# maxdoblas/QuickEd

Hardware: AMD Instinct MI355X
Metric: alignments/sec + GCUPS, 10kb x 10kb 5%-error pairs (higher is better)
Workload: dtype u64; 1 GPU; banded_score, DEVICE-RESIDENT inputs: 100000 pairs/GPU x 10000 bp @ 0.05 error, bandwidth 15 %, seeded generator (SURVEY 8d), ASCII already in HBM when the clock starts, results left in HBM (end-to-end rates: e2e); pairs_per_gpu=100000, length=10000, bandwidth=15, parallelism=pairs sharded over 1 GPU(s), no data-path collective

## Files before the change

### quicked_amd/capi.py

```python
import ctypes as C
import os

import numpy as np

from . import build

QUICKED, WINDOWED, BANDED, HIRSCHBERG = 0, 1, 2, 3
QUICKED_OK, QUICKED_ERROR, QUICKED_FAIL_NON_CONVERGENCE = 0, -1, -2
QUICKED_UNKNOWN_ALGO, QUICKED_EMPTY_SEQUENCE, QUICKED_UNIMPLEMENTED, QUICKED_WIP = -3, -4, -10, 1


class ProfilerCounter(C.Structure):
    _fields_ = [("total", C.c_uint64), ("samples", C.c_uint64), ("min", C.c_uint64), ("max", C.c_uint64),
                ("m_oldM", C.c_double), ("m_newM", C.c_double), ("m_oldS", C.c_double), ("m_newS", C.c_double)]


class Timespec(C.Structure):
    _fields_ = [("tv_sec", C.c_long), ("tv_nsec", C.c_long)]


class ProfilerTimer(C.Structure):
    _fields_ = [("begin_timer", Timespec), ("time_ns", ProfilerCounter), ("accumulated", C.c_uint64)]


# ... 92 lines not shown
    L.quicked_batch_hits.restype = C.c_int
    L.quicked_batch_run_panel.argtypes = [C.c_void_p, C.c_int, C.c_int32, C.c_void_p, C.c_void_p, C.c_void_p, C.c_void_p, C.c_int32, C.c_int]
    L.quicked_batch_run_panel.restype = C.c_int
    L.quicked_batch_panel_results.argtypes = [C.c_void_p, C.c_void_p]
    L.quicked_batch_panel_results.restype = C.c_int
    L.quicked_batch_panel_matrix.argtypes = [C.c_void_p, C.c_void_p, C.c_void_p]
    L.quicked_batch_panel_matrix.restype = C.c_int
    L.quicked_batch_run_panel_all.argtypes = [C.c_void_p, C.c_int, C.c_int32, C.c_void_p, C.c_void_p, C.c_void_p, C.c_void_p, C.c_int32, C.c_int32, C.c_int]
    L.quicked_batch_run_panel_all.restype = C.c_int
    L.quicked_batch_panel_hit_counts.argtypes = [C.c_void_p, C.c_void_p, C.c_void_p]
    L.quicked_batch_panel_hit_counts.restype = C.c_int
    L.quicked_batch_panel_hit_total.argtypes = [C.c_void_p]
    L.quicked_batch_panel_hit_total.restype = C.c_int64
    L.quicked_batch_panel_hits.argtypes = [C.c_void_p, C.c_void_p, C.c_void_p]
    L.quicked_batch_panel_hits.restype = C.c_int
    L.quicked_batch_sync.argtypes = [C.c_void_p]
    L.quicked_batch_scores.argtypes = [C.c_void_p, C.c_void_p, C.c_void_p]
    L.quicked_batch_cigar_bytes.restype = C.c_int64
    L.quicked_batch_cigar_bytes.argtypes = [C.c_void_p]
    L.quicked_batch_cigars.argtypes = [C.c_void_p, C.c_void_p, C.c_void_p]
    L.quicked_batch_counters.argtypes = [C.c_void_p, C.c_void_p]
    L.quicked_batch_kernel_time.argtypes = [C.c_void_p, C.POINTER(C.c_double), C.POINTER(C.c_int64)]
    if hasattr(L, "quicked_batch_kernel_times"):
        L.quicked_batch_kernel_times.argtypes = [C.c_void_p, C.c_void_p, C.c_void_p]
    L.quicked_batch_configure.argtypes = [C.c_void_p, C.c_int, C.c_int]
    L.quicked_batch_check_results.argtypes = [C.c_void_p, C.c_void_p]
    L.quicked_batch_validate.argtypes = [C.c_void_p, C.c_char_p, C.c_int64, C.c_void_p, C.c_void_p]
    L.quicked_batch_configure_tags.argtypes = [C.c_void_p, C.c_int]
    L.quicked_batch_pair_stats.argtypes = [C.c_void_p, C.c_void_p]
    L.quicked_batch_md_bytes.restype = C.c_int64
    L.quicked_batch_md_bytes.argtypes = [C.c_void_p]
    L.quicked_batch_md.argtypes = [C.c_void_p, C.c_void_p, C.c_void_p]
    L.quicked_debug_tag_launches.argtypes = [C.c_void_p]
    L.quicked_wire_words.restype = C.c_int64
    L.quicked_wire_words.argtypes = [C.c_int32, C.c_int]
    L.quicked_wire_pack.argtypes = [C.c_char_p, C.c_int32, C.c_int, C.c_void_p]
    L.quicked_batch_create_packed.restype = C.c_void_p
    L.quicked_batch_create_packed.argtypes = [C.c_int64, C.c_int, C.c_void_p, C.c_void_p, C.c_void_p, C.c_void_p, C.c_void_p, C.c_void_p]
    L.quicked_batch_reload.argtypes = [C.c_void_p, C.c_int64, C.c_void_p, C.c_void_p, C.c_void_p, C.c_void_p, C.c_void_p, C.c_void_p]
    L.quicked_batch_reload_packed.argtypes = [C.c_void_p, C.c_int64, C.c_int, C.c_void_p, C.c_void_p, C.c_void_p, C.c_void_p, C.c_void_p, C.c_void_p]
    L.quicked_batch_fetch.argtypes = [C.c_void_p]
    L.quicked_pool_stats.argtypes = [C.c_void_p]
    if hasattr(L, "quicked_early_finish_stats"):
        L.quicked_early_finish_stats.argtypes = [C.c_void_p]
    L.quicked_batch_cigar_view.argtypes = [C.c_void_p, C.POINTER(C.c_void_p), C.POINTER(C.c_void_p)]
    L.quicked_batch_deferred_pairs.restype = C.c_int64
    L.quicked_batch_deferred_pairs.argtypes = [C.c_void_p]
    L.quicked_wire_pack_pool.argtypes = [C.c_int64, C.c_void_p, C.c_void_p, C.c_void_p, C.c_int, C.c_void_p, C.c_void_p, C.c_int,
                                         C.POINTER(C.c_int64)]
    L.quicked_wire_offsets.restype = C.c_int64
    L.quicked_wire_offsets.argtypes = [C.c_int64, C.c_void_p, C.c_int, C.c_void_p]
    L.quicked_wire_pack_isa.argtypes = [C.c_int]
    L.quicked_host_alloc.restype = C.c_void_p
    L.quicked_host_alloc.argtypes = [C.c_size_t]
    L.quicked_host_free.argtypes = [C.c_void_p]
    L.quicked_host_free.restype = None
    _LIB = L
    return L


def reload_env():
    if _LIB is not None and hasattr(_LIB, "quicked_debug_reload_env"):
        _LIB.quicked_debug_reload_env()


def tag_launches():
    v = np.zeros(2, dtype=np.int64)
    lib().quicked_debug_tag_launches(v.ctypes.data)
    return int(v[0]), int(v[1])


def pool_trim():
    return lib().quicked_pool_trim()


def pool_stats():
    v = np.zeros(8, dtype=np.int64)
    lib().quicked_pool_stats(v.ctypes.data)
    return dict(pool_bytes=int(v[0]), reclaim_events=int(v[1]), sets=int(v[2]), sub_batches=int(v[3]), pool_budget=int(v[4]),
                device_pool_bytes=int(v[5]), contexts=int(v[6]), contexts_leased=int(v[7]))


def early_finish_stats():
    v = np.zeros(4, dtype=np.int64)
    lib().quicked_early_finish_stats(v.ctypes.data)
    return dict(flows=int(v[0]), batches=int(v[1]), merged_flows=int(v[2]), merged_batches=int(v[3]))


def make_params(**kw):
    p = lib().quicked_default_params()
    for k, v in kw.items():
        if k in ("hew_threshold", "hew_percentage"):
            getattr(p, k)[0], getattr(p, k)[1] = v
        else:
            setattr(p, k, v)
    return p


class QuickedException(Exception):
    def __init__(self, status):
        self.status = status
        super().__init__(lib().quicked_status_msg(status).decode())


# ... 399 lines not shown
```

### quicked_amd/csrc/qe_batch.h

```cpp
#pragma once
#include <hip/hip_runtime.h>

#include <condition_variable>
#include <cstdint>
#include <cstring>
#include <memory>
#include <mutex>
#include <vector>

#include "quicked.h"
#include "quicked_batch.h"
#include "qe_types.h"
#include "qe_pool.h"

struct quicked_batch {
    int64_t n = 0;
    int device = 0;
    std::vector<int32_t> p_len, t_len;
    std::vector<int64_t> p_off, t_off;
    std::vector<int64_t> plp_off, plt_off;
    std::vector<int32_t> order;
    uint8_t* arena = nullptr;
    size_t arena_bytes = 0;
    uint8_t *d_asc_p = nullptr, *d_asc_t = nullptr;
// ... 117 lines not shown
    t->accumulated += ns;
    profiler_counter_t* c = &t->time_ns;
    const uint64_t amount = t->accumulated;
    c->total += amount;
    ++c->samples;
    if (c->samples == 1) { c->min = amount; c->max = amount; c->m_oldM = (double)amount; c->m_newM = (double)amount; c->m_oldS = 0.0; }
    else {
        c->min = std::min(c->min, amount); c->max = std::max(c->max, amount);
        c->m_newM = c->m_oldM + ((double)amount - c->m_oldM) / (double)c->samples;
        c->m_newS = c->m_oldS + ((double)amount - c->m_oldM) * ((double)amount - c->m_newM);
        c->m_oldM = c->m_newM; c->m_oldS = c->m_newS;
    }
    t->accumulated = 0;
}

inline double now_ms() { return mono_ms(); }
inline bool trace_on() { return sw_set(Sw::Trace); }
#define QE_TRACE_POINT(name) do { if (qe::trace_on()) { double t__ = qe::now_ms(); fprintf(stderr, "[qe t%03d @%.1f] %-22s +%.3f ms\n", (int)(syscall(SYS_gettid) % 1000), t__, name, t__ - tr_last); tr_last = t__; } } while (0)

struct BoundedRun { const int32_t* max_dist; int32_t max_dist_all; };
struct PanelRun { int32_t n_patterns; const char* pool; const int64_t* off; const int32_t* len; bool matrix; };
struct SearchRun { int mode; const int32_t* max_dist; int32_t max_dist_all; int32_t max_hits = 0; int eq = 0; const PanelRun* panel = nullptr; };
quicked_status_t run_batch(quicked_batch& B, const quicked_params_t& p, bool fetch, const BoundedRun* bd = nullptr, const SearchRun* sr = nullptr);
quicked_status_t fetch_results(quicked_batch& B);
void batch_load(quicked_batch* B, Context& C, int64_t n,
                const char* pattern_pool, const int64_t* pattern_off, const int32_t* pattern_len,
                const char* text_pool, const int64_t* text_off, const int32_t* text_len);
void batch_load_packed(quicked_batch* B, Context& C, int64_t n, int wire,
                       const uint64_t* pattern_words, const int64_t* pattern_word_off, const int32_t* pattern_len,
                       const uint64_t* text_words, const int64_t* text_word_off, const int32_t* text_len);
void batch_quiesce(quicked_batch* B);
void finisher_retire();
quicked_status_t batch_validate(quicked_batch* B, Context& C, const char* cigar_pool, int64_t pool_bytes, const int64_t* cigar_off, int32_t* ok_out);
void early_finish_stats(int64_t stats_out[4]);
int64_t tag_launches(int form);

}
```

### quicked_amd/csrc/qe_capi.cpp

```cpp
#include <hip/hip_runtime.h>

#include <algorithm>
#include <cstdio>
#include <cstdlib>
#include <cstring>
#include <functional>
#include <mutex>
#include <string>
#include <unordered_map>
#include <vector>

#include "qe_batch.h"
#include "qe_panel.h"

#define QE_API extern "C" __attribute__((visibility("default")))

using namespace qe;

QE_API void* quicked_host_alloc(size_t bytes) {
    void* p = nullptr;
    if (hipHostMalloc(&p, bytes, hipHostMallocDefault) != hipSuccess) return nullptr;
    return p;
}
QE_API void quicked_host_free(void* p) { if (p) (void)hipHostFree(p); }
// ... 463 lines not shown
    for (int q = 0; q < 8; ++q) stats_out[q] = 0;
    for (const auto& bk : g_book) stats_out[1] += bk.oom_events.load();
    Context* C = tl_ctx;
    const int dev = C ? C->device : tl_device;
    if (dev >= 0 && dev < QE_MAX_DEVICES) stats_out[5] = (int64_t)g_book[dev].held.load();
    { std::lock_guard<std::mutex> lk(g_ctx_mu); for (const Context* c : g_ctx_all) { ++stats_out[6]; if (c->leased.load()) ++stats_out[7]; } }
    if (!C) return QUICKED_OK;
    stats_out[0] = (int64_t)C->held.load();
    stats_out[2] = C->last_na; stats_out[3] = C->last_sub_batches; stats_out[4] = (int64_t)C->pool_budget;
    return QUICKED_OK;
}

QE_API quicked_status_t quicked_pool_trim(void) {
    finisher_retire();
    ApiScope scope;
    try {
        Context& C = ctx();
        (void)C.release_pools(nullptr, true);
        C.release_small_pinned();
        { std::lock_guard<std::mutex> lk(g_ctx_mu); C.planned = 0; C.wanted = 0; }
        (void)release_unleased(C.device);
        retire_idle_streams(C.device);
        return QUICKED_OK;
    } catch (const HipError& e) {
        fprintf(stderr, "[quicked_hip] HIP error %d (%s) at %s, qe_driver.hip:%d\n", (int)e.e, hipGetErrorString(e.e), e.what, e.line);
        return QUICKED_ERROR;
    }
}

QE_API quicked_status_t quicked_debug_tag_launches(int64_t out[2]) {
    if (!out) return QUICKED_ERROR;
    out[0] = qe::tag_launches(0); out[1] = qe::tag_launches(1);
    return QUICKED_OK;
}

QE_API quicked_status_t quicked_debug_reload_env(void) {
    qe::switches_reload();
    {
        std::lock_guard<std::mutex> lk(qe::g_ctx_mu);
        for (qe::Context* c : qe::g_ctx_all) {
            for (auto& v : c->narrow_off) v = 0;
            for (auto& ring : c->narrow_q) for (auto& v : ring) v = 0;
        }
    }
    return QUICKED_OK;
}

QE_API quicked_status_t quicked_early_finish_stats(int64_t stats_out[4]) {
    qe::early_finish_stats(stats_out);
    return QUICKED_OK;
}

QE_API int64_t quicked_batch_deferred_pairs(quicked_batch_t* batch) { return batch ? batch->res[batch->vis].deferred_pairs : -1; }

QE_API quicked_status_t quicked_batch_counters(quicked_batch_t* batch, int64_t counters_out[8]) {
    memcpy(counters_out, batch->res[batch->vis].counters, sizeof(batch->counters));
    return QUICKED_OK;
}

QE_API bool quicked_check_error(quicked_status_t status) { return status < 0; }

QE_API const char* quicked_status_msg(quicked_status_t status) {
    switch (status) {
        case QUICKED_ERROR: return "ERROR: QuickEd has finished with unspecific error\n";
        case QUICKED_FAIL_NON_CONVERGENCE: return "ERROR: Hirschberg algorithm can not find a middle point of subsequence division!\n";
        case QUICKED_UNIMPLEMENTED: return "ERROR: The algorithm or parameter combination selected is not implemented\n";
// ... 181 lines not shown
```

### quicked_amd/csrc/qe_driver.hip

```cpp
#include <hip/hip_runtime.h>

#include <algorithm>
#include <atomic>
#include <chrono>
#include <condition_variable>
#include <deque>
#include <cstdio>
#include <unistd.h>
#include <cstdlib>
#include <cstring>
#include <functional>
#include <memory>
#include <mutex>
#include <unordered_map>
#include <numeric>
#include <string>
#include <thread>
#include <vector>

#include "quicked.h"
#include "quicked_batch.h"
#include "qe_types.h"
#include "qe_pool.h"
#include "qe_batch.h"
// ... 1583 lines not shown
    }
    HIP_CHECK(hipStreamSynchronize(C.stream));
    QE_TRACE_POINT("load_packed: arrays");
    B->d_wire_p = d_pw; B->d_wire_t = d_tw; B->d_wire_p_off = d_pwo; B->d_wire_t_off = d_two;
    B->unpack_pending = n > 0; B->unpack_event_set = false;
    if (!B->ev_unpacked) HIP_CHECK(hipEventCreateWithFlags(&B->ev_unpacked, hipEventDisableTiming));
    HIP_CHECK(hipStreamSynchronize(C.stream));
}
}

namespace qe {
quicked_status_t fetch_results(quicked_batch& B) { return fetch_pending(B); }
void early_finish_stats(int64_t stats_out[4]) { for (int q = 0; q < 4; ++q) stats_out[q] = g_fin_stats[q].load(); }

quicked_status_t batch_validate(quicked_batch* B, Context& C, const char* cigar_pool, int64_t pool_bytes, const int64_t* cigar_off, int32_t* ok_out) {
    for (int64_t i = 0; i < B->n; ++i) if (cigar_off[i] >= pool_bytes) return QUICKED_ERROR;
    C.sync_all();
    C.phase_u();
    const DevicePool::Mark mk = C.pool_w.mark();
    char* d_pool = C.pool_w.take<char>((size_t)pool_bytes + 16);
    int64_t* d_off = C.pool_w.take<int64_t>((size_t)B->n + 1);
    int32_t* d_ok = C.pool_w.take<int32_t>((size_t)B->n + 1);
    if (pool_bytes > 0) HIP_CHECK(hipMemcpyAsync(d_pool, cigar_pool, (size_t)pool_bytes, hipMemcpyHostToDevice, C.stream));
    HIP_CHECK(hipMemsetAsync(d_pool + pool_bytes, 0, 16, C.stream));
    HIP_CHECK(hipMemcpyAsync(d_off, cigar_off, (size_t)B->n * sizeof(int64_t), hipMemcpyHostToDevice, C.stream));
    const int blocks = (int)((B->n + 63) / 64);
    hipLaunchKernelGGL(k_check_strings, dim3(blocks), dim3(64), 0, C.stream, pair_view(*B, false), (int)B->n,
                       (const char*)d_pool, (const int64_t*)d_off, d_ok);
    HIP_CHECK(hipMemcpyAsync(ok_out, d_ok, (size_t)B->n * sizeof(int32_t), hipMemcpyDeviceToHost, C.stream));
    HIP_CHECK(hipStreamSynchronize(C.stream));
    C.pool_w.release(mk);
    return QUICKED_OK;
}
}
```

### quicked_amd/csrc/qe_kernels.hip

```cpp
#include <type_traits>
#include <hip/hip_runtime.h>
#include "qe_types.h"
#include "qe_bounded.h"
#include "qe_search.h"
#include "qe_panel.h"
#include "qe_tags.h"
#include "qe_check.h"

namespace qe {

#define QE_ONES (~(u64)0)
#define QE_WAVE_IN_BLOCK() ((int)(threadIdx.x >> 6))
#define QE_GROUP_INDEX() ((int)(blockIdx.x * (blockDim.x >> 6) + (threadIdx.x >> 6)))
extern __shared__ uint4 qe_dyn_lds[];

__device__ __forceinline__ u32 lo32(u64 x) { return (u32)x; }
__device__ __forceinline__ u32 hi32(u64 x) { return (u32)(x >> 32); }
__device__ __forceinline__ u64 mk64(u32 lo, u32 hi) { return ((u64)hi << 32) | lo; }

__device__ __forceinline__ int64_t tile_elem(int col, int slot, int nslots) {
    return ((int64_t)(col >> 3) * nslots + slot) * 512 + (col & 7);
}

__device__ __forceinline__ int wave_min(int v) {
#pragma unroll
    for (int o = 32; o > 0; o >>= 1) v = min(v, __shfl_xor(v, o));
    return v;
}
__device__ __forceinline__ int wave_max(int v) {
#pragma unroll
    for (int o = 32; o > 0; o >>= 1) v = max(v, __shfl_xor(v, o));
    return v;
}

__device__ __forceinline__ void block_step(u64 Eq, u64& P, u64& M, u32 PHin, u32 MHin, u64& Ph_raw, u64& Mh_raw) {
    const u64 Xv = Eq | M;
    const u64 Eqc = Eq | (u64)MHin;
    const u64 Xh = (((Eqc & P) + P) ^ P) | Eqc;
// ... 581 lines not shown
            x[k] = (r0 >> sh) | (r1 << (64 - sh));
            y[k] = (r1 >> sh) | (r2 << (64 - sh));
        } else { x[k] = r0; y[k] = r1; }
    }
}

__device__ __forceinline__ void load_planes_ab(const u64* __restrict__ base, int bit, u64& a, u64& b) {
    const int w = bit >> 6, sh = bit & 63, o = sh ? 3 : 0;
    const u64* q = base + 3 * (int64_t)w;
    const u64 a0 = q[0], b0 = q[1], a1 = q[o], b1 = q[o + 1];
    a = (a0 >> sh) | ((a1 << 1) << (63 - sh));
    b = (b0 >> sh) | ((b1 << 1) << (63 - sh));
}

__device__ __forceinline__ void planes_ab_raw(const u64* __restrict__ base, int bit, u64 (&w)[4]) {
    const int o = (bit & 63) ? 3 : 0;
    const u64* q = base + 3 * (int64_t)(bit >> 6);
    w[0] = q[0]; w[1] = q[1]; w[2] = q[o]; w[3] = q[o + 1];
}
__device__ __forceinline__ void planes_ab_finish(const u64 (&w)[4], int bit, u64& a, u64& b) {
    const int sh = bit & 63;
    a = (w[0] >> sh) | ((w[2] << 1) << (63 - sh));
    b = (w[1] >> sh) | ((w[3] << 1) << (63 - sh));
}
struct TbsFetch { int q, Rb, cf_a, cf_b, cl_b; uint4 c0, w0; u64 t[4], p[4]; };

__device__ __forceinline__ int plane_code(const u64* __restrict__ base, int pos) {
    const u64* q = base + 3 * (int64_t)(pos >> 6);
    const int s = pos & 63;
    if ((q[2] >> s) & 1) return 4;
    return (int)(((q[0] >> s) & 1) | (((q[1] >> s) & 1) << 1));
}

__device__ __forceinline__ u32 gather_msb4(u32 x) {
    u32 t = (x << 7) | x;
    t = (x << 14) | t;
    return (x << 21) | t;
}

__global__ __launch_bounds__(256) void k_pack(PackArgs A) {
    const int lane = threadIdx.x & 63;
    const int seq = blockIdx.x * 4 + (threadIdx.x >> 6);
    if (seq >= A.nseq) return;
    const int len = A.len[seq];
    const uint8_t* __restrict__ src = A.asc + A.asc_off[seq];
    u64* __restrict__ dst = A.planes + A.pl_off[seq];
    const int nrows = ((len + 63) >> 6) + 2;
    const int nspan = (nrows + 15) >> 4;
    u32 fl = 0;
    constexpr int UNR = 4;
    constexpr u32 ALL_A = 0x41414141u;
    for (int s0 = 0; s0 < nspan; s0 += UNR) {
        uint4 raw[UNR];
#pragma unroll
        for (int u = 0; u < UNR; ++u) {
            const int pos = (s0 + u) * 1024 + 16 * lane;
            uint4 x = make_uint4(ALL_A, ALL_A, ALL_A, ALL_A);
            if (pos + 16 <= len) {
                if (A.reverse) {
                    uint4 y; __builtin_memcpy(&y, src + (len - 16 - pos), 16);
                    x = make_uint4(__builtin_bswap32(y.w), __builtin_bswap32(y.z), __builtin_bswap32(y.y), __builtin_bswap32(y.x));
                } else {
                    __builtin_memcpy(&x, src + pos, 16);
                }
            } else if (pos < len) {
                u32 wv[4] = {ALL_A, ALL_A, ALL_A, ALL_A};
                for (int i = 0; i < len - pos; ++i) {
                    const u32 c = A.reverse ? src[len - 1 - pos - i] : src[pos + i];
                    wv[i >> 2] = (wv[i >> 2] & ~(0xFFu << (8 * (i & 3)))) | (c << (8 * (i & 3)));
                }
                x = make_uint4(wv[0], wv[1], wv[2], wv[3]);
            }
            raw[u] = x;
        }
#pragma unroll
        for (int u = 0; u < UNR; ++u) {
            const int span = s0 + u;
            if (span >= nspan) break;
            const u32 wv[4] = {raw[u].x, raw[u].y, raw[u].z, raw[u].w};
            u32 accA = 0, accB = 0, accN = 0;
#pragma unroll
            for (int k = 0; k < 4; ++k) {
                const u32 w = wv[k];
                const u32 want = __builtin_amdgcn_perm(0u, 0x47544341u, (w >> 1) & 0x03030303u);
                const u32 y = want ^ (w & 0xDFDFDFDFu);
                const u32 z = ((y & 0x7F7F7F7Fu) + 0x7F7F7F7Fu) | y;
                const u32 ok = ~z & 0x80808080u, bad = z & 0x80808080u;
                accA = (accA >> 4) | (gather_msb4((w << 6) & ok) & 0xF0000000u);
                accB = (accB >> 4) | (gather_msb4((w << 5) & ok) & 0xF0000000u);
                accN = (accN >> 4) | (gather_msb4(bad) & 0xF0000000u);
                if ((w << 2) & ok) fl |= FLAG_NONCANON;
                if (bad) {
                    fl |= FLAG_HAS_N;
                    for (int i = 0; i < 4; ++i)
                        if (((bad >> (8 * i + 7)) & 1) && ((w >> (8 * i)) & 0xFF) != 'N') fl |= FLAG_NONCANON;
                }
            }
            const u32 ab = (accA >> 16) | (accB & 0xFFFF0000u), nn = accN >> 16;
            const u32 ab1 = __shfl_down(ab, 1), nn1 = __shfl_down(nn, 1);
            const u32 a32 = (ab & 0xFFFFu) | (ab1 << 16), b32 = (ab >> 16) | (ab1 & 0xFFFF0000u), n32 = nn | (nn1 << 16);
            const u32 a32h = __shfl_down(a32, 2), b32h = __shfl_down(b32, 2), n32h = __shfl_down(n32, 2);
            const int row = span * 16 + (lane >> 2);
            if ((lane & 3) == 0 && row < nrows) {
                u64* q = dst + 3 * (int64_t)row;
                q[0] = mk64(a32, a32h); q[1] = mk64(b32, b32h); q[2] = mk64(n32, n32h);
            }
        }
    }
    if (A.flags && __any(fl != 0)) {
        u32 f = fl;
#pragma unroll
        for (int o = 32; o > 0; o >>= 1) f |= __shfl_xor(f, o);
        if (lane == 0) atomicOr(&A.flags[seq], f);
    }
}

__device__ __forceinline__ u32 even_bits(u64 x) {
    x &= 0x5555555555555555ull;
    x = (x | (x >> 1)) & 0x3333333333333333ull;
    x = (x | (x >> 2)) & 0x0F0F0F0F0F0F0F0Full;
    x = (x | (x >> 4)) & 0x00FF00FF00FF00FFull;
    x = (x | (x >> 8)) & 0x0000FFFF0000FFFFull;
    x = (x | (x >> 16)) & 0x00000000FFFFFFFFull;
    return (u32)x;
}

__global__ __launch_bounds__(256) void k_unpack_wire(WireArgs A) {
    const int lane = threadIdx.x & 63;
    const int seq = blockIdx.x * 4 + (threadIdx.x >> 6);
    if (seq >= A.nseq) return;
    const int len = A.len[seq];
    const int nw = (len + 63) >> 6;
    const u64* __restrict__ src = A.words + A.w_off[seq];
    u64* __restrict__ dst = A.planes + A.pl_off[seq];
    bool any_n = false;
    for (int r = lane; r < nw + 2; r += 64) {
        u64 a = 0, b = 0, nn = 0;
        if (r < nw) {
            if (A.wire == 3) { a = src[3 * (int64_t)r]; b = src[3 * (int64_t)r + 1]; nn = src[3 * (int64_t)r + 2]; }
            else {
                const int nwords = (len + 31) >> 5;
                const u64 w0 = src[2 * (int64_t)r], w1 = (2 * r + 1 < nwords) ? src[2 * (int64_t)r + 1] : 0;
// ... 3834 lines not shown
```

### quicked_amd/csrc/qe_stages.hip

```cpp
#pragma once

namespace qe {

template <class Args> static Args with_prio(Args a) { a.prio = 1; return a; }

template <typename Kernel, typename Args>
static void launch_groups(Context& C, Kernel kernel, const Args& args, size_t ngroups, int max_waves, size_t lds_per_wave, bool chain = false,
                          size_t pin_override = 0) {
    if (ngroups == 0) return;
    const int wpb = std::min(4, max_waves);
    const unsigned blocks = (unsigned)((ngroups + wpb - 1) / wpb);
    const Chip& chp = chip(C.device);
    size_t pin = ((size_t)blocks * (size_t)std::max(1, C.in_flight) > (size_t)chp.cus) ? (size_t)54 * 1024 : (size_t)84 * 1024;
    if (chain && (size_t)blocks * (size_t)std::max(1, C.in_flight) <= (size_t)chp.cus / 2) pin = (size_t)108 * 1024;
    if (pin_override) pin = pin_override;
    const size_t lds = std::max(pin, lds_per_wave * (size_t)wpb);
    static thread_local std::vector<std::pair<const void*, int>> configured;
    const void* fn = reinterpret_cast<const void*>(kernel);
    if (std::find(configured.begin(), configured.end(), std::make_pair(fn, tl_device)) == configured.end()) {
        HIP_CHECK(hipFuncSetAttribute(fn, hipFuncAttributeMaxDynamicSharedMemorySize, 160 * 1024));
        configured.emplace_back(fn, tl_device);
    }
    hipLaunchKernelGGL(kernel, dim3(blocks), dim3(64 * wpb), lds, C.stream, args);
    HIP_CHECK(hipGetLastError());
}

static void launch_pack(quicked_batch& B, Context& C, bool reversed) {
    if (B.packed) {
        if (!reversed) return;
        const int blocks = (int)((B.n + 3) / 4);
        RevArgs r;
        r.nseq = (int32_t)B.n;
        r.fwd = B.d_pl_p[0]; r.rev = B.d_pl_pr[0]; r.pl_off = B.d_plp_off; r.len = B.d_p_len;
        hipLaunchKernelGGL(k_reverse_planes, dim3(blocks), dim3(256), 0, C.stream, r);
        r.fwd = B.d_pl_t[0]; r.rev = B.d_pl_tr[0]; r.pl_off = B.d_plt_off; r.len = B.d_t_len;
        hipLaunchKernelGGL(k_reverse_planes, dim3(blocks), dim3(256), 0, C.stream, r);
        for (bool& h : B.have_rev) h = true;
        return;
    }
    PackArgs a;
    a.nseq = (int32_t)B.n;
    a.reverse = reversed ? 1 : 0;
    const int q = B.parity;
    a.flags = reversed ? nullptr : B.d_flags[q];
    const int blocks = (int)((B.n + 3) / 4);
    a.asc = B.d_asc_p; a.asc_off = B.d_p_off; a.len = B.d_p_len;
    a.planes = reversed ? B.d_pl_pr[q] : B.d_pl_p[q]; a.pl_off = B.d_plp_off;
    hipLaunchKernelGGL(k_pack, dim3(blocks), dim3(256), 0, C.stream, a);
    a.asc = B.d_asc_t; a.asc_off = B.d_t_off; a.len = B.d_t_len;
    a.planes = reversed ? B.d_pl_tr[q] : B.d_pl_t[q]; a.pl_off = B.d_plt_off;
    hipLaunchKernelGGL(k_pack, dim3(blocks), dim3(256), 0, C.stream, a);
}

struct TaskList {
    std::vector<int32_t> pair, p0, m, t0, n, cutoff, tfin;
    int ngroups() const { return (int)(pair.size() / 64); }
    void push(int32_t pr, int32_t p0_, int32_t m_, int32_t t0_, int32_t n_, int32_t cut, int32_t tf) {
        pair.push_back(pr); p0.push_back(p0_); m.push_back(m_); t0.push_back(t0_); n.push_back(n_);
        cutoff.push_back(cut); tfin.push_back(tf);
    }
    void pad() { while (pair.size() % 64) push(-1, 0, 1, 0, 1, 0, 0); }
};

struct DevTasks {
    TaskView v;
    int32_t *pair, *p0, *m, *t0, *n, *cutoff, *tfin;
};
static void h2d_bytes(void* dst, const void* src, size_t bytes, hipStream_t s) {
    if (bytes == 0) return;
    Context* C = tl_ctx;
    if (C && C->staging && (s == C->sa() || s == C->sw() || s == C->stream_x)) {
        uint8_t* st = C->stage[C->si].take(bytes);
        memcpy(st, src, bytes);
        copy_kernel(dst, st, bytes, s);
        return;
    }
    HIP_CHECK(hipMemcpyAsync(dst, src, bytes, hipMemcpyHostToDevice, s));
}
static DevTasks upload_tasks(const TaskList& L, Context& C) {
    DevTasks d;
    const size_t nt = L.pair.size();
    int32_t* blk = C.scratch_p->take<int32_t>(7 * nt);
    d.pair = blk; d.p0 = blk + nt; d.m = blk + 2 * nt; d.t0 = blk + 3 * nt; d.n = blk + 4 * nt; d.cutoff = blk + 5 * nt; d.tfin = blk + 6 * nt;
    static thread_local std::vector<int32_t> host;
// ... 1219 lines not shown
    uint8_t* h_pool = (uint8_t*)(h_bound + K);
    {
        int64_t at = 0, w = 0;
        for (int p = 0; p < K; ++p) {
            h_asc_off[p] = at; h_pl_off[p] = w; h_len[p] = pr.len[p];
            h_bound[p] = sr.max_dist ? sr.max_dist[p] : sr.max_dist_all;
            memcpy(h_pool + at, pr.pool + pr.off[p], (size_t)pr.len[p]);
            at += pr.len[p]; w += 3 * ((int64_t)(pr.len[p] + 63) / 64 + 2);
        }
    }
    uint8_t* d_blk = C.scratch_p->take<uint8_t>(blk_bytes + 16);
    h2d_bytes(d_blk, host.data(), blk_bytes, C.stream);
    D.d_asc_off = (const int64_t*)d_blk;
    D.d_pl_off = D.d_asc_off + K;
    D.d_len = (const int32_t*)(D.d_pl_off + K);
    D.d_bound = D.d_len + K;
    D.d_pool = (const uint8_t*)(D.d_bound + K);
    D.d_text = C.scratch_p->take<int32_t>(D.nslots);
    h2d(D.d_text, D.text, C.stream);
    return D;
}
static const u64* panel_planes(quicked_batch& B, Context& C, const PanelDev& D, int K, int eq, bool reversed) {
    const size_t plane_words = (size_t)(eq ? iupac_offset((int64_t)D.words3) : (int64_t)D.words3) + 8;
    u64* pl = C.scratch_p->take<u64>(plane_words);
    const int blocks = (K + 3) / 4;
    if (eq) {
        IupacPackArgs a;
        a.nseq = K; a.reverse = reversed ? 1 : 0; a.acgt_only = 0;
        a.asc = D.d_pool; a.asc_off = D.d_asc_off; a.len = D.d_len; a.planes = pl; a.pl_off = D.d_pl_off;
        hipLaunchKernelGGL(k_pack_iupac, dim3(blocks), dim3(256), 0, C.stream, a);
    } else {
        PackArgs a;
        a.nseq = K; a.reverse = reversed ? 1 : 0; a.flags = nullptr;
        a.asc = D.d_pool; a.asc_off = D.d_asc_off; a.len = D.d_len; a.planes = pl; a.pl_off = D.d_pl_off;
        hipLaunchKernelGGL(k_pack, dim3(blocks), dim3(256), 0, C.stream, a);
        if (B.packed) hipLaunchKernelGGL(k_panel_wire_codes, dim3((unsigned)((D.words3 / 3 + 255) / 256)), dim3(256), 0, C.stream, pl, (int64_t)(D.words3 / 3));
    }
    HIP_CHECK(hipGetLastError());
    return (const u64*)pl;
}
static PanelOut run_search_panel(quicked_batch& B, Context& C, const SearchRun& sr) {
    const PanelRun& pr = *sr.panel;
    const int K = pr.n_patterns, eq = sr.eq;
    const bool infix = sr.mode == SEARCH_INFIX;
    PanelOut O;
    const PanelDev D = panel_upload(B, C, sr);
    O.text = D.text;
    if (O.text.empty()) return O;
    const size_t n = (size_t)B.n, nslots = D.nslots, ngroups = D.ngroups;
    const int64_t* d_pl_off = D.d_pl_off;
    const int32_t *d_len = D.d_len, *d_bound = D.d_bound;
    int32_t* d_text = D.d_text;
    auto panel_planes = [&](bool reversed) { return qe::panel_planes(B, C, D, K, eq, reversed); };
    const int want = panel_slices(C, ngroups, K), per_slice = (K + want - 1) / want, nslices = (K + per_slice - 1) / per_slice;
    PanelArgs a{};
    a.pl_m = panel_planes(false); a.m_off = d_pl_off; a.m_len = d_len; a.m_bound = d_bound;
    a.n_members = K; a.per_slice = per_slice;
    a.pl_t = panel_text_planes(B, C, eq, false); a.pl_t_off = B.d_plt_off; a.t_len = B.d_t_len;
    a.nslots = (int32_t)nslots; a.text = d_text; a.mode = sr.mode;
    a.part = C.scratch_p->take<int32_t>(6 * (size_t)nslices * nslots);
    if (pr.matrix) {
        O.d_mscore = C.scratch_p->take<int32_t>(2 * n * (size_t)K);
        O.d_mend = O.d_mscore + n * (size_t)K;
        HIP_CHECK(hipMemsetAsync(O.d_mscore, 0xFF, 2 * n * (size_t)K * sizeof(int32_t), C.stream));
        a.m_score = O.d_mscore; a.m_end = O.d_mend;
    }
    O.d_hits = C.scratch_p->take<int32_t>(6 * n);
// ... 798 lines not shown
```

### quicked_amd/csrc/qe_types.h

```cpp
#pragma once
#include <stdint.h>

namespace qe {

typedef uint64_t u64;
typedef uint32_t u32;

enum : u32 { FLAG_HAS_N = 1u, FLAG_NONCANON = 2u };
enum : int { QE_CP_COLS = 16, QE_CPC = 64 / QE_CP_COLS };
enum : u32 { OP_M = 0, OP_X = 1, OP_I = 2, OP_D = 3 };

struct PairView {
    const uint8_t* asc_p;  const int64_t* asc_p_off;  const int32_t* p_len;
    const uint8_t* asc_t;  const int64_t* asc_t_off;  const int32_t* t_len;
    const u64* pl_p;  const int64_t* pl_p_off;
    const u64* pl_t;  const int64_t* pl_t_off;
    const u32* flags;
};

struct TaskView {
    int32_t ntasks;
    const int32_t* pair;
    const int32_t* p0;  const int32_t* m;
    const int32_t* t0;  const int32_t* n;
    const int32_t* cutoff;
    const int32_t* tfin;
};

struct PackArgs {
    int32_t nseq;
    const uint8_t* asc;  const int64_t* asc_off;  const int32_t* len;
    u64* planes;  const int64_t* pl_off;
    u32* flags;
    int32_t reverse;
};

struct WireArgs {
    int32_t nseq, wire;
    const u64* words;  const int64_t* w_off;  const int32_t* len;
    u64* planes;  const int64_t* pl_off;
    u32* flags;
};
struct RevArgs {
    int32_t nseq;
    const u64* fwd;  u64* rev;  const int64_t* pl_off;  const int32_t* len;
};

struct IupacPackArgs {
    int32_t nseq;
    const uint8_t* asc;  const int64_t* asc_off;  const int32_t* len;
    u64* planes;  const int64_t* pl_off;
    int32_t reverse;
    int32_t acgt_only;
};
struct IupacPlanesArgs {
    int32_t nseq;
    const u64* src;  u64* dst;  const int64_t* pl_off;  const int32_t* len;
    int32_t n_empty;
};

struct BandedArgs {
    PairView P;
    TaskView T;
    uint8_t* ws;  const int64_t* g_ws_off;  const int32_t* g_nslots;  const int32_t* g_nrows;  const int32_t* g_nch;
    uint4* mat;  const int64_t* g_mat_off;
// ... 281 lines not shown
```

Baseline: 22.66 million alignments/s.

## Fuse pattern/text pack launches and vectorize ASCII-to-bitplane classification

Merges the two k_pack launches (pattern and text) into one grid that selects its sequence set by block index. It also rewrites the per-span classification into a shared header that computes the A/B/N bitplanes for 16 bytes with fewer bit operations. The exact flag computation now runs only when a cheap hint says the span may hold non-ACGT or lowercase bytes. Other changes: DPP quad permutes replace the shuffles, full 1 KiB spans skip the bounds checks, and a debug pack entry point is added for testing. This trims launch overhead and ALU work in the pack stage, at the cost of a more intricate bit trick that must stay exact.

```diff
diff --git a/quicked_amd/capi.py b/quicked_amd/capi.py
--- a/quicked_amd/capi.py
+++ b/quicked_amd/capi.py
@@ -148,6 +148,9 @@
     L.quicked_batch_md_bytes.argtypes = [C.c_void_p]
     L.quicked_batch_md.argtypes = [C.c_void_p, C.c_void_p, C.c_void_p]
     L.quicked_debug_tag_launches.argtypes = [C.c_void_p]
+    if hasattr(L, "quicked_debug_pack"):
+        L.quicked_debug_pack.argtypes = [C.c_int64, C.c_void_p, C.c_void_p, C.c_void_p, C.c_void_p, C.c_void_p, C.c_void_p, C.c_int,
+                                         C.c_void_p, C.c_int64, C.c_void_p, C.c_void_p, C.c_int64, C.c_void_p, C.c_void_p]
     L.quicked_wire_words.restype = C.c_int64
     L.quicked_wire_words.argtypes = [C.c_int32, C.c_int]
     L.quicked_wire_pack.argtypes = [C.c_char_p, C.c_int32, C.c_int, C.c_void_p]
@@ -186,6 +189,31 @@
     return int(v[0]), int(v[1])
 
 
+def debug_pack(patterns, texts, reverse=False):
+    assert len(patterns) == len(texts)
+    n = len(patterns)
+
+    def pool_of(seqs):
+        length = np.array([len(s) for s in seqs], dtype=np.int32)
+        off = np.zeros(n, dtype=np.int64)
+        if n:
+            off[1:] = np.cumsum(length[:-1], dtype=np.int64)
+        pool = np.frombuffer(b"".join(seqs) + b"\0", dtype=np.uint8).copy()
+        return pool, off, length, int(sum(3 * ((int(v) + 63) // 64 + 2) for v in length))
+
+    pp, po, pl, pw = pool_of(patterns)
+    tp, to, tl, tw = pool_of(texts)
+    p_words, t_words = np.zeros(pw + 1, dtype=np.uint64), np.zeros(tw + 1, dtype=np.uint64)
+    p_off, t_off = np.zeros(n + 1, dtype=np.int64), np.zeros(n + 1, dtype=np.int64)
+    flags = np.zeros(n + 1, dtype=np.uint32)
+    st = lib().quicked_debug_pack(n, pp.ctypes.data, po.ctypes.data, pl.ctypes.data, tp.ctypes.data, to.ctypes.data, tl.ctypes.data,
+                                  1 if reverse else 0, p_words.ctypes.data, pw, p_off.ctypes.data, t_words.ctypes.data, tw,
+                                  t_off.ctypes.data, flags.ctypes.data)
+    if st < 0:
+        raise QuickedException(st)
+    return p_words[:pw], p_off[:n], t_words[:tw], t_off[:n], flags[:n]
+
+
 def pool_trim():
     return lib().quicked_pool_trim()
 
diff --git a/quicked_amd/csrc/qe_batch.h b/quicked_amd/csrc/qe_batch.h
--- a/quicked_amd/csrc/qe_batch.h
+++ b/quicked_amd/csrc/qe_batch.h
@@ -173,6 +173,8 @@
 void batch_quiesce(quicked_batch* B);
 void finisher_retire();
 quicked_status_t batch_validate(quicked_batch* B, Context& C, const char* cigar_pool, int64_t pool_bytes, const int64_t* cigar_off, int32_t* ok_out);
+quicked_status_t batch_debug_pack(quicked_batch* B, Context& C, bool reversed, uint64_t* p_planes, uint64_t* t_planes,
+                                  int64_t* p_pl_off, int64_t* t_pl_off, uint32_t* flags);
 void early_finish_stats(int64_t stats_out[4]);
 int64_t tag_launches(int form);
 
diff --git a/quicked_amd/csrc/qe_capi.cpp b/quicked_amd/csrc/qe_capi.cpp
--- a/quicked_amd/csrc/qe_capi.cpp
+++ b/quicked_amd/csrc/qe_capi.cpp
@@ -519,6 +519,26 @@
     if (!out) return QUICKED_ERROR;
     out[0] = qe::tag_launches(0); out[1] = qe::tag_launches(1);
     return QUICKED_OK;
+}
+
+QE_API quicked_status_t quicked_debug_pack(int64_t n, const char* pattern_pool, const int64_t* pattern_off, const int32_t* pattern_len,
+                                           const char* text_pool, const int64_t* text_off, const int32_t* text_len, int reversed,
+                                           uint64_t* p_planes, int64_t p_words, int64_t* p_pl_off,
+                                           uint64_t* t_planes, int64_t t_words, int64_t* t_pl_off, uint32_t* flags) {
+    if (n < 0 || !p_planes || !t_planes || !p_pl_off || !t_pl_off || !flags) return QUICKED_ERROR;
+    quicked_batch_t* b = quicked_batch_create(n, pattern_pool, pattern_off, pattern_len, text_pool, text_off, text_len);
+    if (!b) return QUICKED_ERROR;
+    struct Arg { int rev; uint64_t* pp; int64_t pw; int64_t* po; uint64_t* tp; int64_t tw; int64_t* to; uint32_t* fl; }
+        arg{reversed, p_planes, p_words, p_pl_off, t_planes, t_words, t_pl_off, flags};
+    const quicked_status_t st = guard(b, [](quicked_batch* B, void* a) {
+        Arg* x = (Arg*)a;
+        if ((int64_t)B->pl_p_words > x->pw || (int64_t)B->pl_t_words > x->tw) return QUICKED_ERROR;
+        tl_device = B->device;
+        Context& C = ctx();
+        return batch_debug_pack(B, C, x->rev != 0, x->pp, x->tp, x->po, x->to, x->fl);
+    }, &arg);
+    quicked_batch_destroy(b);
+    return st;
 }
 
 QE_API quicked_status_t quicked_debug_reload_env(void) {
diff --git a/quicked_amd/csrc/qe_driver.hip b/quicked_amd/csrc/qe_driver.hip
--- a/quicked_amd/csrc/qe_driver.hip
+++ b/quicked_amd/csrc/qe_driver.hip
@@ -1639,4 +1639,28 @@
     C.pool_w.release(mk);
     return QUICKED_OK;
 }
-}
+
+quicked_status_t batch_debug_pack(quicked_batch* B, Context& C, bool reversed, uint64_t* p_planes, uint64_t* t_planes,
+                                  int64_t* p_pl_off, int64_t* t_pl_off, uint32_t* flags) {
+    if (B->packed) return QUICKED_UNIMPLEMENTED;
+    C.sync_all();
+    C.phase_u();
+    B->parity = 0;
+    const size_t n = (size_t)B->n;
+    if (n == 0) return QUICKED_OK;
+    u64* const d_p = reversed ? B->d_pl_pr[0] : B->d_pl_p[0];
+    u64* const d_t = reversed ? B->d_pl_tr[0] : B->d_pl_t[0];
+    HIP_CHECK(hipMemsetAsync(d_p, 0xFF, B->pl_p_words * sizeof(u64), C.stream));
+    HIP_CHECK(hipMemsetAsync(d_t, 0xFF, B->pl_t_words * sizeof(u64), C.stream));
+    HIP_CHECK(hipMemsetAsync(B->d_flags[0], 0, n * sizeof(u32), C.stream));
+    launch_pack(*B, C, reversed, true);
+    HIP_CHECK(hipGetLastError());
+    HIP_CHECK(hipMemcpyAsync(p_planes, d_p, B->pl_p_words * sizeof(u64), hipMemcpyDeviceToHost, C.stream));
+    HIP_CHECK(hipMemcpyAsync(t_planes, d_t, B->pl_t_words * sizeof(u64), hipMemcpyDeviceToHost, C.stream));
+    HIP_CHECK(hipMemcpyAsync(flags, B->d_flags[0], n * sizeof(u32), hipMemcpyDeviceToHost, C.stream));
+    HIP_CHECK(hipStreamSynchronize(C.stream));
+    memcpy(p_pl_off, B->plp_off.data(), n * sizeof(int64_t));
+    memcpy(t_pl_off, B->plt_off.data(), n * sizeof(int64_t));
+    return QUICKED_OK;
+}
+}
diff --git a/quicked_amd/csrc/qe_kernels.hip b/quicked_amd/csrc/qe_kernels.hip
--- a/quicked_amd/csrc/qe_kernels.hip
+++ b/quicked_amd/csrc/qe_kernels.hip
@@ -4,6 +4,7 @@
 #include "qe_bounded.h"
 #include "qe_search.h"
 #include "qe_panel.h"
+#include "qe_pack.h"
 #include "qe_tags.h"
 #include "qe_check.h"
 
@@ -651,82 +652,90 @@
     return (int)(((q[0] >> s) & 1) | (((q[1] >> s) & 1) << 1));
 }
 
-__device__ __forceinline__ u32 gather_msb4(u32 x) {
-    u32 t = (x << 7) | x;
-    t = (x << 14) | t;
-    return (x << 21) | t;
+static_assert(PACK_HAS_N == FLAG_HAS_N && PACK_NONCANON == FLAG_NONCANON, "qe_pack.h's flag bits are the batch's");
+template <int CTRL> __device__ __forceinline__ u32 quad_perm(u32 x) {
+    return (u32)__builtin_amdgcn_mov_dpp((int)x, CTRL, 0xF, 0xF, true);
+}
+
+template <bool GUARDED>
+__device__ __forceinline__ void pack_span(const uint4& x, u64* __restrict__ dst, int span, int lane, int nrows, bool want_flags, u32& fl) {
+    const u32 w[4] = {x.x, x.y, x.z, x.w};
+    u32 a, b, n, hint;
+    pack_classify16(w, a, b, n, hint);
+    if (want_flags && __any(hint != 0)) fl |= pack_flags16(w);
+    const u32 ab = a | (b << 16);
+    const u32 ab1 = quad_perm<0xF5>(ab), n1 = quad_perm<0xF5>(n);
+    const u32 a32 = __builtin_amdgcn_perm(ab1, ab, 0x05040100u), b32 = __builtin_amdgcn_perm(ab1, ab, 0x07060302u), n32 = n | (n1 << 16);
+    const u32 a32h = quad_perm<0xAA>(a32), b32h = quad_perm<0xAA>(b32), n32h = quad_perm<0xAA>(n32);
+    const int row = span * 16 + (lane >> 2);
+    if ((lane & 3) == 0 && (!GUARDED || row < nrows)) {
+        u64* q = dst + 3 * (int64_t)row;
+        q[0] = mk64(a32, a32h); q[1] = mk64(b32, b32h); q[2] = mk64(n32, n32h);
+    }
+}
+template <bool REVERSE> __device__ __forceinline__ uint4 pack_load16(const uint8_t* p) {
+    uint4 y; __builtin_memcpy(&y, p, 16);
+    if (REVERSE) y = make_uint4(__builtin_bswap32(y.w), __builtin_bswap32(y.z), __builtin_bswap32(y.y), __builtin_bswap32(y.x));
+    return y;
+}
+
+template <bool REVERSE>
+__device__ __forceinline__ u32 pack_sequence(const uint8_t* __restrict__ src, int len, u64* __restrict__ dst, int lane, bool want_flags) {
+    const int nrows = ((len + 63) >> 6) + 2;
+    const int nspan = (nrows + 15) >> 4;
+    const int nfull = len >> 10;
+    u32 fl = 0;
+    constexpr int UNR = 4;
+    int s0 = 0;
+    const u32 lane_off = REVERSE ? 1008u - 16u * (u32)lane : 16u * (u32)lane;
+    for (; s0 + UNR <= nfull; s0 += UNR) {
+        uint4 raw[UNR];
+#pragma unroll
+        for (int u = 0; u < UNR; ++u) {
+            const uint8_t* base = src + (REVERSE ? len - 1024 * (s0 + u + 1) : 1024 * (s0 + u));
+            raw[u] = pack_load16<REVERSE>(base + lane_off);
+        }
+#pragma unroll
+        for (int u = 0; u < UNR; ++u) pack_span<false>(raw[u], dst, s0 + u, lane, nrows, want_flags, fl);
+    }
+    for (; s0 < nspan; s0 += UNR) {
+        uint4 raw[UNR];
+#pragma unroll
+        for (int u = 0; u < UNR; ++u) {
+            const int pos = (s0 + u) * 1024 + 16 * lane;
+            uint4 x = make_uint4(PACK_FILL, PACK_FILL, PACK_FILL, PACK_FILL);
+            if (pos + 16 <= len) x = pack_load16<REVERSE>(src + (REVERSE ? len - 16 - pos : pos));
+            else if (pos < len) {
+                u32 wv[4];
+                pack_fetch16(src, len, pos, REVERSE, wv);
+                x = make_uint4(wv[0], wv[1], wv[2], wv[3]);
+            }
+            raw[u] = x;
+        }
+#pragma unroll
+        for (int u = 0; u < UNR; ++u) {
+            if (s0 + u >= nspan) break;
+            pack_span<true>(raw[u], dst, s0 + u, lane, nrows, want_flags, fl);
+        }
+    }
+    return fl;
 }
 
 __global__ __launch_bounds__(256) void k_pack(PackArgs A) {
     const int lane = threadIdx.x & 63;
-    const int seq = blockIdx.x * 4 + (threadIdx.x >> 6);
+    const int per_set = (A.nseq + 3) >> 2;
+    const bool second = (int)blockIdx.x >= per_set;
+    const int seq = ((int)blockIdx.x - (second ? per_set : 0)) * 4 + __builtin_amdgcn_readfirstlane((int)(threadIdx.x >> 6));
     if (seq >= A.nseq) return;
-    const int len = A.len[seq];
-    const uint8_t* __restrict__ src = A.asc + A.asc_off[seq];
-    u64* __restrict__ dst = A.planes + A.pl_off[seq];
-    const int nrows = ((len + 63) >> 6) + 2;
-    const int nspan = (nrows + 15) >> 4;
-    u32 fl = 0;
-    constexpr int UNR = 4;
-    constexpr u32 ALL_A = 0x41414141u;
-    for (int s0 = 0; s0 < nspan; s0 += UNR) {
-        uint4 raw[UNR];
-#pragma unroll
-        for (int u = 0; u < UNR; ++u) {
-            const int pos = (s0 + u) * 1024 + 16 * lane;
-            uint4 x = make_uint4(ALL_A, ALL_A, ALL_A, ALL_A);
-            if (pos + 16 <= len) {
-                if (A.reverse) {
-                    uint4 y; __builtin_memcpy(&y, src + (len - 16 - pos), 16);
-                    x = make_uint4(__builtin_bswap32(y.w), __builtin_bswap32(y.z), __builtin_bswap32(y.y), __builtin_bswap32(y.x));
-                } else {
-                    __builtin_memcpy(&x, src + pos, 16);
-                }
-            } else if (pos < len) {
-                u32 wv[4] = {ALL_A, ALL_A, ALL_A, ALL_A};
-                for (int i = 0; i < len - pos; ++i) {
-                    const u32 c = A.reverse ? src[len - 1 - pos - i] : src[pos + i];
-                    wv[i >> 2] = (wv[i >> 2] & ~(0xFFu << (8 * (i & 3)))) | (c << (8 * (i & 3)));
-                }
-                x = make_uint4(wv[0], wv[1], wv[2], wv[3]);
-            }
-            raw[u] = x;
-        }
-#pragma unroll
-        for (int u = 0; u < UNR; ++u) {
-            const int span = s0 + u;
-            if (span >= nspan) break;
-            const u32 wv[4] = {raw[u].x, raw[u].y, raw[u].z, raw[u].w};
-            u32 accA = 0, accB = 0, accN = 0;
-#pragma unroll
-            for (int k = 0; k < 4; ++k) {
-                const u32 w = wv[k];
-                const u32 want = __builtin_amdgcn_perm(0u, 0x47544341u, (w >> 1) & 0x03030303u);
-                const u32 y = want ^ (w & 0xDFDFDFDFu);
-                const u32 z = ((y & 0x7F7F7F7Fu) + 0x7F7F7F7Fu) | y;
-                const u32 ok = ~z & 0x80808080u, bad = z & 0x80808080u;
-                accA = (accA >> 4) | (gather_msb4((w << 6) & ok) & 0xF0000000u);
-                accB = (accB >> 4) | (gather_msb4((w << 5) & ok) & 0xF0000000u);
-                accN = (accN >> 4) | (gather_msb4(bad) & 0xF0000000u);
-                if ((w << 2) & ok) fl |= FLAG_NONCANON;
-                if (bad) {
-                    fl |= FLAG_HAS_N;
-                    for (int i = 0; i < 4; ++i)
-                        if (((bad >> (8 * i + 7)) & 1) && ((w >> (8 * i)) & 0xFF) != 'N') fl |= FLAG_NONCANON;
-                }
-            }
-            const u32 ab = (accA >> 16) | (accB & 0xFFFF0000u), nn = accN >> 16;
-            const u32 ab1 = __shfl_down(ab, 1), nn1 = __shfl_down(nn, 1);
-            const u32 a32 = (ab & 0xFFFFu) | (ab1 << 16), b32 = (ab >> 16) | (ab1 & 0xFFFF0000u), n32 = nn | (nn1 << 16);
-            const u32 a32h = __shfl_down(a32, 2), b32h = __shfl_down(b32, 2), n32h = __shfl_down(n32, 2);
-            const int row = span * 16 + (lane >> 2);
-            if ((lane & 3) == 0 && row < nrows) {
-                u64* q = dst + 3 * (int64_t)row;
-                q[0] = mk64(a32, a32h); q[1] = mk64(b32, b32h); q[2] = mk64(n32, n32h);
-            }
-        }
-    }
-    if (A.flags && __any(fl != 0)) {
+    const int32_t* __restrict__ lens = second ? A.set[1].len : A.set[0].len;
+    const int64_t* __restrict__ asc_off = second ? A.set[1].asc_off : A.set[0].asc_off;
+    const int64_t* __restrict__ pl_off = second ? A.set[1].pl_off : A.set[0].pl_off;
+    const int len = lens[seq];
+    const uint8_t* __restrict__ src = (second ? A.set[1].asc : A.set[0].asc) + asc_off[seq];
+    u64* __restrict__ dst = (second ? A.set[1].planes : A.set[0].planes) + pl_off[seq];
+    const bool want_flags = A.flags != nullptr;
+    const u32 fl = A.reverse ? pack_sequence<true>(src, len, dst, lane, want_flags) : pack_sequence<false>(src, len, dst, lane, want_flags);
+    if (want_flags && __any(fl != 0)) {
         u32 f = fl;
 #pragma unroll
         for (int o = 32; o > 0; o >>= 1) f |= __shfl_xor(f, o);
diff --git a/quicked_amd/csrc/qe_pack.h b/quicked_amd/csrc/qe_pack.h
--- /dev/null
+++ b/quicked_amd/csrc/qe_pack.h
@@ -0,0 +1,76 @@
+#pragma once
+#include <stdint.h>
+
+#if defined(__HIPCC__) || defined(__CUDACC__)
+#define QE_K_HD __host__ __device__ __forceinline__
+#else
+#define QE_K_HD inline
+#endif
+
+namespace qe {
+
+typedef uint32_t u32;
+enum : u32 { PACK_HAS_N = 1u, PACK_NONCANON = 2u };
+
+QE_K_HD u32 pack_perm(u32 hi, u32 lo, u32 sel) {
+#if defined(__HIP_DEVICE_COMPILE__)
+    return __builtin_amdgcn_perm(hi, lo, sel);
+#else
+    u32 r = 0;
+    for (int k = 0; k < 4; ++k) {
+        const u32 c = (sel >> (8 * k)) & 0xFFu;
+        const u32 byte = c < 4u ? (lo >> (8 * c)) & 0xFFu : c < 8u ? (hi >> (8 * (c - 4u))) & 0xFFu : 0u;
+        r |= byte << (8 * k);
+    }
+    return r;
+#endif
+}
+QE_K_HD u32 pack_gather8(u32 u) {
+    const u32 t = u | (u << 7);
+    return t | (t << 14);
+}
+
+enum : u32 { PACK_FILL = 0x41414141u };
+
+QE_K_HD u32 pack_not_acgt(u32 w) {
+    const u32 want = pack_perm(0u, 0x47544341u, (w >> 1) & 0x03030303u);
+    const u32 y = want ^ (w & 0xDFDFDFDFu);
+    const u32 y7 = want ^ (w & 0x5F5F5F5Fu);
+    return ((y7 + 0x7F7F7F7Fu) | y) & 0x80808080u;
+}
+
+QE_K_HD void pack_classify16(const u32 (&w)[4], u32& a, u32& b, u32& n, u32& hint) {
+    const u32 n0 = pack_gather8((pack_not_acgt(w[0]) >> 4) | pack_not_acgt(w[1]));
+    const u32 n1 = pack_gather8((pack_not_acgt(w[2]) >> 4) | pack_not_acgt(w[3]));
+    n = pack_perm(n1, n0, 0x0C0C0703u);
+    const u32 m0 = (w[0] & 0x06060606u) | ((w[1] << 4) & 0x60606060u), m1 = (w[2] & 0x06060606u) | ((w[3] << 4) & 0x60606060u);
+    const u32 a0 = pack_gather8(m0 & 0x22222222u), a1 = pack_gather8(m1 & 0x22222222u);
+    const u32 b0 = pack_gather8(m0 & 0x44444444u), b1 = pack_gather8(m1 & 0x44444444u);
+    a = (((a0 >> 22) & 0xFFu) | ((a1 >> 14) & 0xFF00u)) & ~n;
+    b = (((b0 >> 23) & 0xFFu) | ((b1 >> 15) & 0xFF00u)) & ~n;
+    hint = ((w[0] | w[1] | w[2] | w[3]) & 0x20202020u) | n;
+}
+
+QE_K_HD u32 pack_flags16(const u32 (&w)[4]) {
+    u32 fl = 0;
+    for (int k = 0; k < 4; ++k) {
+        const u32 bad = pack_not_acgt(w[k]);
+        if ((w[k] << 2) & ~bad & 0x80808080u) fl |= PACK_NONCANON;
+        if (bad) {
+            fl |= PACK_HAS_N;
+            for (int i = 0; i < 4; ++i)
+                if (((bad >> (8 * i + 7)) & 1u) && ((w[k] >> (8 * i)) & 0xFFu) != 'N') fl |= PACK_NONCANON;
+        }
+    }
+    return fl;
+}
+
+QE_K_HD void pack_fetch16(const uint8_t* src, int len, int pos, bool reverse, u32 (&w)[4]) {
+    w[0] = w[1] = w[2] = w[3] = PACK_FILL;
+    for (int i = 0; i < 16 && pos + i < len; ++i) {
+        const u32 c = reverse ? src[len - 1 - pos - i] : src[pos + i];
+        w[i >> 2] = (w[i >> 2] & ~(0xFFu << (8 * (i & 3)))) | (c << (8 * (i & 3)));
+    }
+}
+
+}
diff --git a/quicked_amd/csrc/qe_stages.hip b/quicked_amd/csrc/qe_stages.hip
--- a/quicked_amd/csrc/qe_stages.hip
+++ b/quicked_amd/csrc/qe_stages.hip
@@ -25,7 +25,7 @@
     HIP_CHECK(hipGetLastError());
 }
 
-static void launch_pack(quicked_batch& B, Context& C, bool reversed) {
+static void launch_pack(quicked_batch& B, Context& C, bool reversed, bool flags_of_reversed = false) {
     if (B.packed) {
         if (!reversed) return;
         const int blocks = (int)((B.n + 3) / 4);
@@ -42,14 +42,11 @@
     a.nseq = (int32_t)B.n;
     a.reverse = reversed ? 1 : 0;
     const int q = B.parity;
-    a.flags = reversed ? nullptr : B.d_flags[q];
+    a.flags = (reversed && !flags_of_reversed) ? nullptr : B.d_flags[q];
     const int blocks = (int)((B.n + 3) / 4);
-    a.asc = B.d_asc_p; a.asc_off = B.d_p_off; a.len = B.d_p_len;
-    a.planes = reversed ? B.d_pl_pr[q] : B.d_pl_p[q]; a.pl_off = B.d_plp_off;
-    hipLaunchKernelGGL(k_pack, dim3(blocks), dim3(256), 0, C.stream, a);
-    a.asc = B.d_asc_t; a.asc_off = B.d_t_off; a.len = B.d_t_len;
-    a.planes = reversed ? B.d_pl_tr[q] : B.d_pl_t[q]; a.pl_off = B.d_plt_off;
-    hipLaunchKernelGGL(k_pack, dim3(blocks), dim3(256), 0, C.stream, a);
+    a.set[0] = PackSet{B.d_asc_p, B.d_p_off, B.d_p_len, reversed ? B.d_pl_pr[q] : B.d_pl_p[q], B.d_plp_off};
+    a.set[1] = PackSet{B.d_asc_t, B.d_t_off, B.d_t_len, reversed ? B.d_pl_tr[q] : B.d_pl_t[q], B.d_plt_off};
+    hipLaunchKernelGGL(k_pack, dim3(2 * blocks), dim3(256), 0, C.stream, a);
 }
 
 struct TaskList {
@@ -1335,7 +1332,8 @@
     } else {
         PackArgs a;
         a.nseq = K; a.reverse = reversed ? 1 : 0; a.flags = nullptr;
-        a.asc = D.d_pool; a.asc_off = D.d_asc_off; a.len = D.d_len; a.planes = pl; a.pl_off = D.d_pl_off;
+        a.set[0] = PackSet{D.d_pool, D.d_asc_off, D.d_len, pl, D.d_pl_off};
+        a.set[1] = a.set[0];
         hipLaunchKernelGGL(k_pack, dim3(blocks), dim3(256), 0, C.stream, a);
         if (B.packed) hipLaunchKernelGGL(k_panel_wire_codes, dim3((unsigned)((D.words3 / 3 + 255) / 256)), dim3(256), 0, C.stream, pl, (int64_t)(D.words3 / 3));
     }
diff --git a/quicked_amd/csrc/qe_types.h b/quicked_amd/csrc/qe_types.h
--- a/quicked_amd/csrc/qe_types.h
+++ b/quicked_amd/csrc/qe_types.h
@@ -27,10 +27,13 @@
     const int32_t* tfin;
 };
 
+struct PackSet {
+    const uint8_t* asc;  const int64_t* asc_off;  const int32_t* len;
+    u64* planes;  const int64_t* pl_off;
+};
 struct PackArgs {
     int32_t nseq;
-    const uint8_t* asc;  const int64_t* asc_off;  const int32_t* len;
-    u64* planes;  const int64_t* pl_off;
+    PackSet set[2];
     u32* flags;
     int32_t reverse;
 };
```

After: 23.65 million alignments/s, median of 6. 4.4% higher.
